# CenekAlbl/mvus

Hardware: AMD Instinct MI355X
Metric: residuals/sec (higher is better)
Workload: dtype f64; 1 GPU; BASELINE configs[2]: 32 cams x 504399 obs (504399 per GPU), rolling shutter on, 5003 spline control points, 15297 params, 1008798 residual rows; step = 1 trust-region trial (residual+Jacobian, LM normal equations + Schur solve, trial residual); solver=lm, parallelism=time-shard x1

## Files before the change

### mvus_amd/csrc/ba_rcs.hip.h

```cpp
#pragma once

namespace mvus {

constexpr int kRcsSP = 9;
constexpr int kRcsFactorThreads = 64 * (kRcsSP + 3);
constexpr int kRcsTrsmWaves = 4;

struct RcsView {
  double* Simg;
  double* Tsc;
  double* x;
  int nn, nbk;
};

__host__ __device__ __forceinline__ long long rcs_blk(int i, int j) { return ((long long)i * (i + 1) / 2 + j) * 256; }
__host__ __device__ inline size_t rcs_doubles(int nn) { const int nbk = (nn + 15) / 16; return (size_t)rcs_blk(nbk + 1, 0); }
__device__ __forceinline__ bcr_d4 rcs_load(const double* __restrict__ p) { return *reinterpret_cast<const bcr_d4*>(p); }
__device__ __forceinline__ void rcs_store(double* __restrict__ p, bcr_d4 v) { *reinterpret_cast<bcr_d4*>(p) = v; }
__device__ __forceinline__ bcr_d4 rcs_mma(bcr_d4 p, bcr_d4 q, bcr_d4 acc) {
#pragma unroll
  for (int s = 0; s < 4; ++s) acc = __builtin_amdgcn_mfma_f64_16x16x4f64(p[s], q[s], acc, 0, 0, 0);
  return acc;
}
__device__ __forceinline__ bcr_d4 rcs_matvec(bcr_d4 img, double w) {
  bcr_d4 out;
#pragma unroll
  for (int r = 0; r < 4; ++r) {
    double v = img[r] * w;
    v += dpp_shift<0x111, 0xF>(v, 0.0);
    v += dpp_shift<0x112, 0xF>(v, 0.0);
    v += dpp_shift<0x114, 0xF>(v, 0.0);
    v += dpp_shift<0x118, 0xF>(v, 0.0);
    out[r] = v;
  }
  return out;
}

struct RcsPivotChain { double d, r, e; bool bad; };
template <int J> __device__ __forceinline__ double rcs_bcast(double v) {
  const int lo = __builtin_amdgcn_mov_dpp(__double2loint(v), 0x150 + J, 0xf, 0xf, true);
  const int hi = __builtin_amdgcn_mov_dpp(__double2hiint(v), 0x150 + J, 0xf, 0xf, true);
  return __hiloint2double(hi, lo);
}
template <int STAGE, int J> __device__ __forceinline__ void rcs_chain_stage(RcsPivotChain& c, const double (&a)[16]) {
  if constexpr (STAGE == 0) { double d = rcs_bcast<J>(a[J]); c.bad |= !(d > 0.0); c.d = d > 0.0 ? d : 1.0; }
  else if constexpr (STAGE == 1) c.r = __builtin_amdgcn_rcp(c.d);
  else if constexpr (STAGE == 2 || STAGE == 4) c.e = 2.0 - c.d * c.r;
  else if constexpr (STAGE == 3 || STAGE == 5) c.r = c.r * c.e;
}
template <int FROM, int KN> struct RcsChainRest {
  static __device__ __forceinline__ void run(RcsPivotChain& c, const double (&a)[16]) {
    if constexpr (FROM <= 5) { rcs_chain_stage<FROM, KN>(c, a); RcsChainRest<FROM + 1, KN>::run(c, a); }
  }
};
template <int K, int J> struct RcsColOps {
  static __device__ __forceinline__ void run(double (&a)[16], double (&x)[16], double ta, double tx, double m, RcsPivotChain& c) {
    if constexpr (J < 16) {
      double mn = 0.0;
      if constexpr (J + 1 < 16) mn = rcs_bcast<J + 1>(a[K]);
      a[J] -= ta * m;
      x[J] -= tx * m;
      rcs_chain_stage<J - (K + 1), K + 1>(c, a);
      asm volatile("" : "+v"(a[J]), "+v"(x[J]), "+v"(c.d), "+v"(c.r), "+v"(c.e), "+v"(mn));
      __builtin_amdgcn_sched_barrier(0);
      RcsColOps<K, J + 1>::run(a, x, ta, tx, mn, c);
    }
  }
};
template <int K> struct RcsCols {
  static __device__ __forceinline__ void run(double (&a)[16], double (&x)[16], double (&rd)[16], RcsPivotChain& c) {
    const double r = c.r;
    rd[K] = r;
    if constexpr (K + 1 < 16) {
      const double m0 = rcs_bcast<K + 1>(a[K]);
      const double ta = a[K] * r, tx = x[K] * r;
      RcsColOps<K, K + 1>::run(a, x, ta, tx, m0, c);
      RcsChainRest<(15 - K < 6 ? 15 - K : 6), K + 1>::run(c, a);
      __builtin_amdgcn_sched_barrier(0);
      RcsCols<K + 1>::run(a, x, rd, c);
    }
  }
};
__device__ __forceinline__ void rcs_ldl16(double (&a)[16], double (&x)[16], double (&rd)[16], int lane, int* __restrict__ fail) {
  RcsPivotChain c{0.0, 0.0, 0.0, false};
  RcsChainRest<0, 0>::run(c, a);
  RcsCols<0>::run(a, x, rd, c);
  if (c.bad && lane == 0) fail[0] = 2;
}

__global__ __launch_bounds__(256) void k_rcs_finish(NEView ne, int ncols, int nslab, double lambda, const double* __restrict__ Gp, RcsView rv,
                                                    unsigned* __restrict__ flags) {
  constexpr int kT = 32, kRowsPer = 4, kRowStep = 8;
  const int r0 = threadIdx.x / kT, c = threadIdx.x % kT;
  const int b = blockIdx.x * kT + c;
  const long long stride = (long long)ne.CB * ncols;
  const int nn = ne.CB, npad = rv.nbk * 16;
  if (blockIdx.y == gridDim.y - 1) {
    if (blockIdx.x == 0 && threadIdx.x == 0) flags[0] = 0u;
    if (r0 != 0 || b >= npad) return;
    double gr = 0.0;
    if (b < nn) {
      for (int sl = 0; sl < nslab; sl += 8) {
        double t[8];
#pragma unroll
        for (int u = 0; u < 8; ++u) t[u] = sl + u < nslab ? Gp[(sl + u) * stride + (long long)b * ncols + ne.CB] : 0.0;
#pragma unroll
        for (int u = 0; u < 8; ++u) gr += t[u];
      }
    }
    const double val = b < nn ? ne.gc[b] - gr : 0.0;
    double* blk = rv.Simg + rcs_blk(rv.nbk, b / 16);
    const int cc = b % 16;
    for (int lr = 0; lr < 16; ++lr) blk[((cc % 4) * 16 + lr) * 4 + cc / 4] = lr == 0 ? val : 0.0;
    return;
  }
  if (blockIdx.x > blockIdx.y) return;
  double gsum[kRowsPer];
  long long goff[kRowsPer];
#pragma unroll
  for (int q = 0; q < kRowsPer; ++q) {
    const int a = blockIdx.y * kT + r0 + kRowStep * q;
    const int hi = a / kGemmT >= b / kGemmT ? a : b, lo = a / kGemmT >= b / kGemmT ? b : a;
    goff[q] = (a < nn && b < nn) ? (long long)hi * ncols + lo : -1;
    gsum[q] = 0.0;
  }
  for (int sl = 0; sl < nslab; sl += 8) {
    double t[8][kRowsPer];
#pragma unroll
    for (int u = 0; u < 8; ++u)
#pragma unroll
      for (int q = 0; q < kRowsPer; ++q) t[u][q] = (sl + u < nslab && goff[q] >= 0) ? Gp[(sl + u) * stride + goff[q]] : 0.0;
#pragma unroll
    for (int u = 0; u < 8; ++u)
#pragma unroll
      for (int q = 0; q < kRowsPer; ++q) gsum[q] += t[u][q];
  }
#pragma unroll
  for (int q = 0; q < kRowsPer; ++q) {
    const int a = blockIdx.y * kT + r0 + kRowStep * q;
    if (a >= npad || b >= npad || a / 16 < b / 16) continue;
    double v = a == b ? 1.0 : 0.0;
    if (a < nn && b < nn) {
      v = -gsum[q];
      if (a / ne.B == b / ne.B) {
        const int cam = a / ne.B;
        double h = ne.A[((long long)cam * ne.B + a % ne.B) * ne.B + b % ne.B];
        if (a == b) h += lambda * (h > 0.0 ? h : 1.0);
        v += h;
      }
    }
    const int cc = b % 16;
    rv.Simg[rcs_blk(a / 16, b / 16) + ((cc % 4) * 16 + a % 16) * 4 + cc / 4] = v;
  }
}

using rcs_u4 = __attribute__((ext_vector_type(4))) unsigned;
struct RcsWide { rcs_u4 a, b; };
__device__ __forceinline__ __amdgpu_buffer_rsrc_t rcs_rsrc(double* p, size_t doubles) {
  return __builtin_amdgcn_make_buffer_rsrc(p, 0, (int)(doubles * sizeof(double)), 0x00020000);
}
__device__ __forceinline__ void rcs_store_sc1(__amdgpu_buffer_rsrc_t r, long long dbl_off, bcr_d4 v) {
  RcsWide w;
  __builtin_memcpy(&w, &v, sizeof(w));
  __builtin_amdgcn_raw_buffer_store_b128(w.a, r, (int)(dbl_off * 8), 0, 16);
  __builtin_amdgcn_raw_buffer_store_b128(w.b, r, (int)(dbl_off * 8 + 16), 0, 16);
}
__device__ __forceinline__ bcr_d4 rcs_load_sc1(__amdgpu_buffer_rsrc_t r, long long dbl_off) {
  RcsWide w;
  w.a = __builtin_amdgcn_raw_buffer_load_b128(r, (int)(dbl_off * 8), 0, 16);
  w.b = __builtin_amdgcn_raw_buffer_load_b128(r, (int)(dbl_off * 8 + 16), 0, 16);
  bcr_d4 v;
  __builtin_memcpy(&v, &w, sizeof(v));
  return v;
}
__device__ __forceinline__ double rcs_load1_sc1(__amdgpu_buffer_rsrc_t r, long long dbl_off) {
  using u2 = __attribute__((ext_vector_type(2))) unsigned;
  const u2 w = __builtin_amdgcn_raw_buffer_load_b64(r, (int)(dbl_off * 8), 0, 16);
  double v;
  __builtin_memcpy(&v, &w, sizeof(v));
  return v;
}
__device__ __forceinline__ void rcs_store1_sc1(__amdgpu_buffer_rsrc_t r, long long dbl_off, double v) {
  using u2 = __attribute__((ext_vector_type(2))) unsigned;
  u2 w;
  __builtin_memcpy(&w, &v, sizeof(w));
  __builtin_amdgcn_raw_buffer_store_b64(w, r, (int)(dbl_off * 8), 0, 16);
}
constexpr unsigned kRcsSpinLimit = 1u << 21;
constexpr int kFailHandover = kFailHandoverCode;

template <int J> struct RcsXtTimes {
  static __device__ __forceinline__ double run(const double* __restrict__ col, double w, double acc) {
    if constexpr (J < 16) return RcsXtTimes<J + 1>::run(col, w, acc + col[J] * rcs_bcast<J>(w));
    else return acc;
  }
};
__device__ __forceinline__ double rcs_xt_times(const double* __restrict__ col, double w) { return RcsXtTimes<0>::run(col, w, 0.0); }
__device__ __forceinline__ void rcs_part_product(const bcr_d4 (&sl)[kRcsSP], int k, const double* __restrict__ xi, double* __restrict__ out, int lr, int lk) {
  const double xv = xi[lr];
#pragma unroll
  for (int kk = 0; kk < kRcsSP; ++kk) {
    if (kk != k) continue;
    const bcr_d4 y = rcs_matvec(sl[kk], xv);
    if (lr == 15) {
#pragma unroll
      for (int r = 0; r < 4; ++r) out[lk + 4 * r] = y[r];
    }
  }
}

__device__ __forceinline__ void rcs_pivot_role(int nc, int* __restrict__ fail, double* __restrict__ Dm, double* __restrict__ Xb, double* __restrict__ rdb) {
  const int lane = threadIdx.x & 63;
  __builtin_amdgcn_s_setprio(3);
  for (int k = 0; k < nc; ++k) {
    if (k == 0) lds_barrier();
    double a[16], x[16], rd[16];
    int lr = lane & 15;
    asm volatile("" : "+v"(lr));
#pragma unroll
    for (int j = 0; j < 16; ++j) {
      a[j] = Dm[lr * 17 + j];
      x[j] = j == lr ? 1.0 : 0.0;
    }
    rcs_ldl16(a, x, rd, lane, fail);
    if (lane < 16) {
#pragma unroll
      for (int q = 0; q < 4; ++q) rcs_store(Xb + k * 256 + lane * 16 + 4 * q, bcr_d4{x[4 * q], x[4 * q + 1], x[4 * q + 2], x[4 * q + 3]});
    }
    if (lane == 0) {
#pragma unroll
      for (int q = 0; q < 4; ++q) rcs_store(rdb + k * 16 + 4 * q, bcr_d4{rd[4 * q], rd[4 * q + 1], rd[4 * q + 2], rd[4 * q + 3]});
    }
    lds_barrier();
    lds_barrier();
  }
}

__device__ __forceinline__ void rcs_trsm_role(RcsView rv, int c0, int nc, unsigned* __restrict__ flags, int* __restrict__ fail, double* __restrict__ xch,
                                              int* __restrict__ abort_s, unsigned spin_limit) {
  const int lane = threadIdx.x & 63, wave = __builtin_amdgcn_readfirstlane(threadIdx.x >> 6), lk = lane >> 4;
  const int c1 = c0 + nc, gi = c1 + (int)blockIdx.x - 1;
  const size_t tot = rcs_doubles(rv.nn);
  const __amdgpu_buffer_rsrc_t rS = rcs_rsrc(rv.Simg, tot), rT = rcs_rsrc(rv.Tsc, tot);
  constexpr int kSlots = (kRcsSP + kRcsTrsmWaves - 1) / kRcsTrsmWaves;
  bcr_d4 s[kSlots];
  const bcr_d4 zero{0.0, 0.0, 0.0, 0.0};
#pragma unroll
  for (int u = 0; u < kSlots; ++u) {
    const int jl = wave + kRcsTrsmWaves * u;
    s[u] = jl < nc ? rcs_load(rv.Simg + rcs_blk(gi, c0 + jl) + lane * 4) : zero;
  }
  if (threadIdx.x == 0) *abort_s = 0;
  lds_barrier();
#pragma unroll
  for (int k = 0; k < kRcsSP; ++k) {
    if (k >= nc) continue;
    if (threadIdx.x == 0 && *abort_s == 0) {
      const unsigned want = (unsigned)(c0 * 16 + k + 1);
      unsigned spins = 0;
      while (__hip_atomic_load(flags, __ATOMIC_RELAXED, __HIP_MEMORY_SCOPE_AGENT) < want) {
        __builtin_amdgcn_s_sleep(8);
        if (++spins > spin_limit) { *abort_s = 1; fail[0] = kFailHandover; fail[2] = 1; break; }
      }
    }
    lds_barrier();
    const bool dead = *abort_s != 0;
    bcr_d4 tj[kSlots];
    bool up[kSlots];
#pragma unroll
    for (int u = 0; u < kSlots; ++u) {
      const int jl = wave + kRcsTrsmWaves * u;
      up[u] = jl > k && jl < nc && !dead;
      tj[u] = up[u] ? rcs_load_sc1(rS, rcs_blk(c0 + jl, c0 + k) + lane * 4) : zero;
    }
    if (wave == k % kRcsTrsmWaves && !dead) {
      const bcr_d4 xi = rcs_load_sc1(rS, rcs_blk(c0 + k, c0 + k) + lane * 4);
      bcr_d4 nrd;
#pragma unroll
      for (int r = 0; r < 4; ++r) nrd[r] = -rcs_load1_sc1(rT, rcs_blk(c0 + k, c0 + k) + lk + 4 * r);
      const bcr_d4 t = rcs_mma(xi, s[k / kRcsTrsmWaves], zero);
      s[k / kRcsTrsmWaves] = t;
      rcs_store(xch + (k & 1) * 256 + lane * 4, t * nrd);
    }
    lds_barrier();
    if (k + 1 >= nc || dead) continue;
    const bcr_d4 sc = rcs_load(xch + (k & 1) * 256 + lane * 4);
#pragma unroll
    for (int q = 0; q < 4; ++q)
#pragma unroll
      for (int u = 0; u < kSlots; ++u)
        if (up[u]) s[u] = __builtin_amdgcn_mfma_f64_16x16x4f64(tj[u][q], sc[q], s[u], 0, 0, 0);
  }
#pragma unroll
  for (int u = 0; u < kSlots; ++u) {
    const int jl = wave + kRcsTrsmWaves * u;
    if (jl >= nc) continue;
    bcr_d4 sc;
#pragma unroll
    for (int r = 0; r < 4; ++r) sc[r] = -rcs_load1_sc1(rT, rcs_blk(c0 + jl, c0 + jl) + lk + 4 * r) * s[u][r];
    rcs_store(rv.Simg + rcs_blk(gi, c0 + jl) + lane * 4, s[u]);
    rcs_store(rv.Tsc + rcs_blk(gi, c0 + jl) + lane * 4, sc);
  }
}

__device__ __forceinline__ void rcs_publisher_role(RcsView rv, int c0, int nc, unsigned* __restrict__ flags, const double* __restrict__ Xb,
                                                   const double* __restrict__ rdb, const double* __restrict__ panel) {
  const int lane = threadIdx.x & 63, lr = lane & 15, lk = lane >> 4;
  const size_t tot = rcs_doubles(rv.nn);
  const __amdgpu_buffer_rsrc_t rS = rcs_rsrc(rv.Simg, tot), rT = rcs_rsrc(rv.Tsc, tot);
  lds_barrier();
  for (int k = 0; k < nc; ++k) {
    lds_barrier();
    if (k > 0) {
      asm volatile("s_waitcnt vmcnt(0)" ::: "memory");
      if (lane == 0) __hip_atomic_store(flags, (unsigned)(c0 * 16 + k), __ATOMIC_RELAXED, __HIP_MEMORY_SCOPE_AGENT);
    }
    lds_barrier();
    bcr_d4 xi;
#pragma unroll
    for (int r = 0; r < 4; ++r) xi[r] = Xb[k * 256 + (lk + 4 * r) * 16 + lr];
    rcs_store_sc1(rS, rcs_blk(c0 + k, c0 + k) + lane * 4, xi);
    if (lane < 16) rcs_store1_sc1(rT, rcs_blk(c0 + k, c0 + k) + lane, rdb[k * 16 + lane]);
    for (int jl = k + 1; jl < nc; ++jl) rcs_store_sc1(rS, rcs_blk(c0 + jl, c0 + k) + lane * 4, rcs_load(panel + jl * 256 + lane * 4));
    asm volatile("s_waitcnt lgkmcnt(0)" ::: "memory");
  }
  asm volatile("s_waitcnt vmcnt(0)" ::: "memory");
  if (lane == 0) __hip_atomic_store(flags, (unsigned)(c0 * 16 + nc), __ATOMIC_RELAXED, __HIP_MEMORY_SCOPE_AGENT);
}

__global__ __launch_bounds__(kRcsFactorThreads) void k_rcs_factor(RcsView rv, int c0, int* __restrict__ fail, int last, double* __restrict__ pc,
                                                                  unsigned* __restrict__ flags, unsigned spin_limit) {
  __shared__ double Dm[16 * 17];
  __shared__ __attribute__((aligned(32))) double Xb[kRcsSP * 256];
  __shared__ __attribute__((aligned(32))) double rdb[kRcsSP * 16];
  __shared__ __attribute__((aligned(32))) double panel[(kRcsSP + 1) * 256];
  __shared__ int abort_s;
  const int lane = threadIdx.x & 63, wave = __builtin_amdgcn_readfirstlane(threadIdx.x >> 6), lr = lane & 15, lk = lane >> 4;
  const int nc = min(kRcsSP, rv.nbk - c0), R = rv.nbk;
  if (blockIdx.x > 0) {
    if (wave < kRcsTrsmWaves) rcs_trsm_role(rv, c0, nc, flags, fail, panel, &abort_s, spin_limit);
    return;
  }
  if (wave == kRcsSP + 2) {
    if (gridDim.x > 1) rcs_publisher_role(rv, c0, nc, flags, Xb, rdb, panel);
    else { lds_barrier(); for (int k = 0; k < nc; ++k) { lds_barrier(); lds_barrier(); } }
    if (last) { lds_barrier(); for (int i = 0; i < nc; ++i) { lds_barrier(); lds_barrier(); } }
    return;
  }
  __shared__ double u0[kRcsSP * 16];
  __shared__ double part[kRcsSP * kRcsSP * 16];
  __shared__ double xs[kRcsSP * 16];
  if (wave == kRcsSP + 1) {
    rcs_pivot_role(nc, fail, Dm, Xb, rdb);
    if (!last || c0 > 0)
      for (int k = 0; k < nc; ++k) {
        bcr_d4 xi;
#pragma unroll
        for (int r = 0; r < 4; ++r) xi[r] = Xb[k * 256 + (lk + 4 * r) * 16 + lr];
        rcs_store(rv.Simg + rcs_blk(c0 + k, c0 + k) + lane * 4, xi);
        if (lane < 16) rv.Tsc[rcs_blk(c0 + k, c0 + k) + lane] = rdb[k * 16 + lane];
      }
    if (!last) return;
    __builtin_amdgcn_s_setprio(0);
    lds_barrier();
    for (int i = nc - 1; i >= 0; --i) {
      double xi = 0.0;
      if (lane < 16) {
        double w = u0[i * 16 + lane];
        for (int ip = i + 1; ip < nc; ++ip) w -= part[(ip * kRcsSP + i) * 16 + lane];
        w *= rdb[i * 16 + lane];
        xi = rcs_xt_times(Xb + i * 256 + lane * 16, w);
        xs[i * 16 + lane] = xi;
      }
      lds_barrier();
      lds_barrier();
    }
    if (lane < 16)
      for (int k = 0; k < nc; ++k) {
        const int a = (c0 + k) * 16 + lane;
        const double v = xs[k * 16 + lane];
        rv.x[a] = v;
        if (a < rv.nn) pc[a] = -v;
      }
    return;
  }
  const int il = wave;
  const bool has = il <= nc, isR = il == nc;
  const int gi = isR ? R : c0 + il;
  bcr_d4 sl[kRcsSP];
  const bcr_d4 zero{0.0, 0.0, 0.0, 0.0};
#pragma unroll
  for (int jl = 0; jl < kRcsSP; ++jl) sl[jl] = (has && jl < nc && (isR || jl <= il)) ? rcs_load(rv.Simg + rcs_blk(gi, c0 + jl) + lane * 4) : zero;
  if (wave == 0) {
#pragma unroll
    for (int r = 0; r < 4; ++r) Dm[(lk + 4 * r) * 17 + lr] = sl[0][r];
  }
  lds_barrier();
#pragma unroll
  for (int k = 0; k < kRcsSP; ++k) {
    if (k < nc) {
      lds_barrier();
      const bool act = has && il > k;
      const bool owner = act && il == k + 1 && !isR && k + 1 < nc;
      if (owner) __builtin_amdgcn_s_setprio(2);
      bcr_d4 sc = zero;
      if (act) {
        bcr_d4 xi;
#pragma unroll
        for (int r = 0; r < 4; ++r) xi[r] = Xb[k * 256 + (lk + 4 * r) * 16 + lr];
        const bcr_d4 t = rcs_mma(xi, sl[k], zero);
        sl[k] = t;
#pragma unroll
        for (int r = 0; r < 4; ++r) sc[r] = -rdb[k * 16 + lk + 4 * r] * t[r];
        rcs_store(panel + il * 256 + lane * 4, t);
      }
      const int kn = k + 1 < kRcsSP ? k + 1 : 0;
      if (owner) {
        sl[kn] = rcs_mma(sl[k], sc, sl[kn]);
#pragma unroll
        for (int r = 0; r < 4; ++r) Dm[(lk + 4 * r) * 17 + lr] = sl[kn][r];
        __builtin_amdgcn_s_setprio(0);
      }
      lds_barrier();
      {
        bcr_d4 tj[kRcsSP];
        bool up[kRcsSP];
#pragma unroll
        for (int jl = k + 1; jl < kRcsSP; ++jl) {
          up[jl] = jl < nc && act && (isR || jl <= il) && !(owner && jl == k + 1);
          tj[jl] = up[jl] ? rcs_load(panel + jl * 256 + lane * 4) : zero;
        }
#pragma unroll
        for (int q = 0; q < 4; ++q)
#pragma unroll
          for (int jl = k + 1; jl < kRcsSP; ++jl)
            if (up[jl]) sl[jl] = __builtin_amdgcn_mfma_f64_16x16x4f64(tj[jl][q], sc[q], sl[jl], 0, 0, 0);
      }
    }
  }
  if (has && (!last || c0 > 0)) {
#pragma unroll
  for (int k = 0; k < kRcsSP; ++k) {
    if (k < nc && il > k) {
      bcr_d4 sc;
#pragma unroll
      for (int r = 0; r < 4; ++r) sc[r] = -rdb[k * 16 + lk + 4 * r] * sl[k][r];
      rcs_store(rv.Simg + rcs_blk(gi, c0 + k) + lane * 4, sl[k]);
      rcs_store(rv.Tsc + rcs_blk(gi, c0 + k) + lane * 4, sc);
    }
  }
  }
  if (!last) return;
  if (has && isR && lr == 0) {
#pragma unroll
    for (int k = 0; k < kRcsSP; ++k)
      if (k < nc)
#pragma unroll
        for (int r = 0; r < 4; ++r) u0[k * 16 + lk + 4 * r] = sl[k][r];
  }
  lds_barrier();
  for (int i = nc - 1; i >= 0; --i) {
    const bool mine = has && !isR && il > i;
    int kd = mine ? 2 * i - il : -1;
    if (kd >= 0) rcs_part_product(sl, kd, xs + il * 16, part + (il * kRcsSP + kd) * 16, lr, lk);
    lds_barrier();
    kd = (has && !isR && il == i) ? i - 1 : (mine ? 2 * i - il - 1 : -1);
    if (kd >= 0) rcs_part_product(sl, kd, xs + il * 16, part + (il * kRcsSP + kd) * 16, lr, lk);
    lds_barrier();
  }
}

__host__ __device__ inline int rcs_stage_doubles(int nc) { return nc * 256 + nc * 16 + nc * (nc - 1) / 2 * 256; }
__device__ __forceinline__ int rcs_tri(int j, int k) { return j * (j - 1) / 2 + k; }
template <int NWAVES>
__device__ __forceinline__ void rcs_stage(const RcsView& rv, int c0, int nc, double* __restrict__ st, int lane, int wave) {
  constexpr int kMaxBlk = kRcsSP + kRcsSP * (kRcsSP - 1) / 2, kPer = (kMaxBlk + NWAVES - 1) / NWAVES;
  double* rds = st + nc * 256;
  double* ts = rds + nc * 16;
  const int nblk = nc + nc * (nc - 1) / 2;
  bcr_d4 v[kPer];
  double rdv[kPer];
  int dst[kPer];
#pragma unroll
  for (int u = 0; u < kPer; ++u) {
    const int t = wave + NWAVES * u;
    dst[u] = -1; rdv[u] = 0.0;
    if (t < nc) {
      v[u] = rcs_load(rv.Simg + rcs_blk(c0 + t, c0 + t) + lane * 4);
      if (lane < 16) rdv[u] = rv.Tsc[rcs_blk(c0 + t, c0 + t) + lane];
      dst[u] = t * 256;
    } else if (t < nblk) {
      const int e = t - nc;
      int j = (int)((1.0f + sqrtf(1.0f + 8.0f * (float)e)) * 0.5f);
      while (j * (j - 1) / 2 > e) --j;
      while (j * (j + 1) / 2 <= e) ++j;
      const int k = e - j * (j - 1) / 2;
      v[u] = rcs_load(rv.Simg + rcs_blk(c0 + j, c0 + k) + lane * 4);
      dst[u] = (int)(ts - st) + e * 256;
    }
  }
#pragma unroll
  for (int u = 0; u < kPer; ++u) {
    const int t = wave + NWAVES * u;
    if (dst[u] >= 0) rcs_store(st + dst[u] + lane * 4, v[u]);
    if (t < nc && lane < 16) rds[t * 16 + lane] = rdv[u];
  }
}

__global__ __launch_bounds__(64 * kRcsTrsmWaves) void k_rcs_trsm(RcsView rv, int c0) {
  extern __shared__ __attribute__((aligned(32))) double rcs_lds[];
  const int lane = threadIdx.x & 63, wave = __builtin_amdgcn_readfirstlane(threadIdx.x >> 6), lk = lane >> 4;
  const int nc = min(kRcsSP, rv.nbk - c0), c1 = c0 + nc;
  rcs_stage<kRcsTrsmWaves>(rv, c0, nc, rcs_lds, lane, wave);
  const double* rds = rcs_lds + nc * 256;
  const double* ts = rds + nc * 16;
  double* xch = rcs_lds + rcs_stage_doubles(nc);
  const int gi = c1 + blockIdx.x;
  constexpr int kSlots = (kRcsSP + kRcsTrsmWaves - 1) / kRcsTrsmWaves;
  bcr_d4 s[kSlots];
  const bcr_d4 zero{0.0, 0.0, 0.0, 0.0};
#pragma unroll
  for (int u = 0; u < kSlots; ++u) {
    const int jl = wave + kRcsTrsmWaves * u;
    s[u] = jl < nc ? rcs_load(rv.Simg + rcs_blk(gi, c0 + jl) + lane * 4) : zero;
  }
  lds_barrier();
#pragma unroll
  for (int k = 0; k < kRcsSP; ++k) {
    if (k >= nc) continue;
    if (wave == k % kRcsTrsmWaves) {
      const bcr_d4 t = rcs_mma(rcs_load(rcs_lds + k * 256 + lane * 4), s[k / kRcsTrsmWaves], zero);
      s[k / kRcsTrsmWaves] = t;
      bcr_d4 sc;
#pragma unroll
      for (int r = 0; r < 4; ++r) sc[r] = -rds[k * 16 + lk + 4 * r] * t[r];
      rcs_store(xch + (k & 1) * 256 + lane * 4, sc);
    }
    lds_barrier();
    if (k + 1 >= nc) continue;
    const bcr_d4 sc = rcs_load(xch + (k & 1) * 256 + lane * 4);
    bcr_d4 tj[kSlots];
    bool up[kSlots];
#pragma unroll
    for (int u = 0; u < kSlots; ++u) {
      const int jl = wave + kRcsTrsmWaves * u;
      up[u] = jl > k && jl < nc;
      tj[u] = up[u] ? rcs_load(ts + rcs_tri(jl, k) * 256 + lane * 4) : zero;
    }
#pragma unroll
    for (int q = 0; q < 4; ++q)
#pragma unroll
      for (int u = 0; u < kSlots; ++u)
        if (up[u]) s[u] = __builtin_amdgcn_mfma_f64_16x16x4f64(tj[u][q], sc[q], s[u], 0, 0, 0);
  }
#pragma unroll
  for (int u = 0; u < kSlots; ++u) {
    const int jl = wave + kRcsTrsmWaves * u;
    if (jl >= nc) continue;
    bcr_d4 sc;
#pragma unroll
    for (int r = 0; r < 4; ++r) sc[r] = -rds[jl * 16 + lk + 4 * r] * s[u][r];
    rcs_store(rv.Simg + rcs_blk(gi, c0 + jl) + lane * 4, s[u]);
    rcs_store(rv.Tsc + rcs_blk(gi, c0 + jl) + lane * 4, sc);
  }
}

__global__ __launch_bounds__(256) void k_rcs_syrk(RcsView rv, int c0) {
  const int lane = threadIdx.x & 63, wave = __builtin_amdgcn_readfirstlane(threadIdx.x >> 6);
  const int nc = min(kRcsSP, rv.nbk - c0), c1 = c0 + nc, m = rv.nbk - c1;
  const int t = blockIdx.x * 4 + wave, ntri = m * (m + 1) / 2;
  if (t >= ntri + m) return;
  int il, jl;
  if (t < ntri) {
    il = (int)((sqrt(8.0 * t + 1.0) - 1.0) * 0.5);
    while ((il + 1) * (il + 2) / 2 <= t) ++il;
    while (il * (il + 1) / 2 > t) --il;
    jl = t - il * (il + 1) / 2;
  } else { il = m; jl = t - ntri; }
  const int gi = c1 + il, gj = c1 + jl;
  double* blk = rv.Simg + rcs_blk(gi, gj) + lane * 4;
  bcr_d4 acc = rcs_load(blk);
  bcr_d4 pj[kRcsSP], qi[kRcsSP];
#pragma unroll
  for (int k = 0; k < kRcsSP; ++k) {
    if (k >= nc) continue;
    pj[k] = rcs_load(rv.Simg + rcs_blk(gj, c0 + k) + lane * 4);
    qi[k] = rcs_load(rv.Tsc + rcs_blk(gi, c0 + k) + lane * 4);
  }
#pragma unroll
  for (int k = 0; k < kRcsSP; ++k)
    if (k < nc) acc = rcs_mma(pj[k], qi[k], acc);
  rcs_store(blk, acc);
}

constexpr int kRcsBackWaves = 16;
__host__ __device__ inline int rcs_backsub_doubles(int nbk) { return nbk * 16 + (1 + kRcsBackWaves) * kRcsSP * 16 + rcs_stage_doubles(kRcsSP); }
__global__ __launch_bounds__(64 * kRcsBackWaves) void k_rcs_backsub(RcsView rv, double* __restrict__ pc, int Kfirst) {
  extern __shared__ __attribute__((aligned(32))) double rcs_lds[];
  const int lane = threadIdx.x & 63, wave = __builtin_amdgcn_readfirstlane(threadIdx.x >> 6), lr = lane & 15, lk = lane >> 4;
  const int nbk = rv.nbk, R = nbk;
  double* xs = rcs_lds;
  double* u = xs + nbk * 16;
  double* up = u + kRcsSP * 16;
  double* st = up + kRcsBackWaves * kRcsSP * 16;
  for (int a = (Kfirst + 1) * kRcsSP * 16 + threadIdx.x; a < nbk * 16; a += 64 * kRcsBackWaves) xs[a] = rv.x[a];
  constexpr int kBatch = 4;
  for (int K = Kfirst; K >= 0; --K) {
    const int c0 = K * kRcsSP, nc = min(kRcsSP, nbk - c0), c1 = c0 + nc;
    lds_barrier();
    double* rds = st + nc * 256;
    double* ts = rds + nc * 16;
    const int nblk = nc + nc * (nc - 1) / 2;
    constexpr int kPer = (kRcsSP + kRcsSP * (kRcsSP - 1) / 2 + kRcsBackWaves - 1) / kRcsBackWaves;
    bcr_d4 sv[kPer];
    double srd[kPer];
    int sdst[kPer];
#pragma unroll
    for (int q = 0; q < kPer; ++q) {
      const int t = wave + kRcsBackWaves * q;
      sdst[q] = -1; srd[q] = 0.0;
      if (t < nc) {
        sv[q] = rcs_load(rv.Simg + rcs_blk(c0 + t, c0 + t) + lane * 4);
        if (lane < 16) srd[q] = rv.Tsc[rcs_blk(c0 + t, c0 + t) + lane];
        sdst[q] = t * 256;
      } else if (t < nblk) {
        const int e = t - nc;
        int j = (int)((1.0f + sqrtf(1.0f + 8.0f * (float)e)) * 0.5f);
        while (j * (j - 1) / 2 > e) --j;
        while (j * (j + 1) / 2 <= e) ++j;
        sv[q] = rcs_load(rv.Simg + rcs_blk(c0 + j, c0 + e - j * (j - 1) / 2) + lane * 4);
        sdst[q] = (int)(ts - st) + e * 256;
      }
    }
    double tR = 0.0;
    if (threadIdx.x < nc * 16) {
      const int jl = threadIdx.x / 16, row = threadIdx.x % 16;
      tR = rv.Simg[rcs_blk(R, c0 + jl) + ((row & 3) * 16) * 4 + (row >> 2)];
    }
    const int nitem = (nbk - c1) * nc;
    bcr_d4 img[kBatch];
    double xv[kBatch];
#pragma unroll
    for (int q = 0; q < kBatch; ++q) {
      const int it = min(wave + kRcsBackWaves * q, max(nitem - 1, 0)), i = c1 + it / nc, jl = it % nc;
      img[q] = nitem > 0 ? rcs_load(rv.Simg + rcs_blk(i, c0 + jl) + lane * 4) : bcr_d4{0.0, 0.0, 0.0, 0.0};
      xv[q] = nitem > 0 ? xs[i * 16 + lr] : 0.0;
    }
#pragma unroll
    for (int q = 0; q < kPer; ++q) {
      const int t = wave + kRcsBackWaves * q;
      if (sdst[q] >= 0) rcs_store(st + sdst[q] + lane * 4, sv[q]);
      if (t < nc && lane < 16) rds[t * 16 + lane] = srd[q];
    }
    for (int e = lane; e < nc * 16; e += 64) up[wave * kRcsSP * 16 + e] = 0.0;
    lds_wave_sync();
    for (int it0 = wave; it0 < nitem; it0 += kRcsBackWaves * kBatch) {
      if (it0 != wave) {
#pragma unroll
        for (int q = 0; q < kBatch; ++q) {
          const int it = min(it0 + kRcsBackWaves * q, nitem - 1), i = c1 + it / nc, jl = it % nc;
          img[q] = rcs_load(rv.Simg + rcs_blk(i, c0 + jl) + lane * 4);
          xv[q] = xs[i * 16 + lr];
        }
      }
#pragma unroll
      for (int q = 0; q < kBatch; ++q) {
        const int it = it0 + kRcsBackWaves * q;
        if (it >= nitem) continue;
        const int jl = it % nc;
        const bcr_d4 y = rcs_matvec(img[q], xv[q]);
        if (lr == 15) {
#pragma unroll
          for (int r = 0; r < 4; ++r) up[wave * kRcsSP * 16 + jl * 16 + lk + 4 * r] += y[r];
        }
      }
    }
    lds_barrier();
    if (threadIdx.x < nc * 16) {
      double v = tR;
#pragma unroll
      for (int w = 0; w < kRcsBackWaves; ++w) v -= up[w * kRcsSP * 16 + threadIdx.x];
      u[threadIdx.x] = v;
    }
    lds_barrier();
    for (int k = nc - 1; k >= 0; --k) {
      if (wave == 0) {
        const bcr_d4 y = rcs_matvec(rcs_load(st + k * 256 + lane * 4), rds[k * 16 + lr] * u[k * 16 + lr]);
        if (lr == 15) {
#pragma unroll
          for (int r = 0; r < 4; ++r) xs[(c0 + k) * 16 + lk + 4 * r] = y[r];
        }
      }
      lds_barrier();
      if (wave < k) {
        const bcr_d4 y = rcs_matvec(rcs_load(ts + rcs_tri(k, wave) * 256 + lane * 4), xs[(c0 + k) * 16 + lr]);
        if (lr == 15) {
#pragma unroll
          for (int r = 0; r < 4; ++r) u[wave * 16 + lk + 4 * r] -= y[r];
        }
      }
      lds_barrier();
    }
  }
  const int top = min((Kfirst + 1) * kRcsSP * 16, rv.nn);
  for (int a = threadIdx.x; a < top; a += 64 * kRcsBackWaves) pc[a] = -xs[a];
}

}
```

Measured before the change: 1.132 billion residuals/s.

## Move next-pivot diagonal update into pivot wave and remap wave roles across SIMDs

```diff
diff --git a/mvus_amd/csrc/ba_rcs.hip.h b/mvus_amd/csrc/ba_rcs.hip.h
--- a/mvus_amd/csrc/ba_rcs.hip.h
+++ b/mvus_amd/csrc/ba_rcs.hip.h
@@ -209,8 +209,10 @@
   }
 }
 
-__device__ __forceinline__ void rcs_pivot_role(int nc, int* __restrict__ fail, double* __restrict__ Dm, double* __restrict__ Xb, double* __restrict__ rdb) {
-  const int lane = threadIdx.x & 63;
+__device__ __forceinline__ void rcs_pivot_role(int nc, int* __restrict__ fail, double* __restrict__ Dm, double* __restrict__ Xb, double* __restrict__ rdb,
+                                               const double* __restrict__ stg, double* __restrict__ panel) {
+  const int lane = threadIdx.x & 63, lk = lane >> 4;
+  const bcr_d4 zero{0.0, 0.0, 0.0, 0.0};
   __builtin_amdgcn_s_setprio(3);
   for (int k = 0; k < nc; ++k) {
     if (k == 0) lds_barrier();
@@ -232,6 +234,20 @@
       for (int q = 0; q < 4; ++q) rcs_store(rdb + k * 16 + 4 * q, bcr_d4{rd[4 * q], rd[4 * q + 1], rd[4 * q + 2], rd[4 * q + 3]});
     }
     lds_barrier();
+    if (k + 1 < nc) {
+      const int lc = lane & 15;
+      bcr_d4 xi, sc;
+#pragma unroll
+      for (int r = 0; r < 4; ++r) xi[r] = Xb[k * 256 + (lk + 4 * r) * 16 + lc];
+      const bcr_d4 u = rcs_load(stg + lane * 4), dn = rcs_load(stg + 256 + lane * 4);
+      const bcr_d4 t = rcs_mma(xi, u, zero);
+#pragma unroll
+      for (int r = 0; r < 4; ++r) sc[r] = -rdb[k * 16 + lk + 4 * r] * t[r];
+      rcs_store(panel + (k + 1) * 256 + lane * 4, t);
+      const bcr_d4 d = rcs_mma(t, sc, dn);
+#pragma unroll
+      for (int r = 0; r < 4; ++r) Dm[(lk + 4 * r) * 17 + lc] = d[r];
+    }
     lds_barrier();
   }
 }
@@ -328,19 +344,44 @@
   if (lane == 0) __hip_atomic_store(flags, (unsigned)(c0 * 16 + nc), __ATOMIC_RELAXED, __HIP_MEMORY_SCOPE_AGENT);
 }
 
+__device__ __forceinline__ int rcs_factor_role(int* __restrict__ simd_of) {
+  constexpr int kWaves = kRcsSP + 3;
+  constexpr int kRole[kWaves] = {kRcsSP + 1, kRcsSP + 2, 0, kRcsSP, 5, 1, 8, 4, 3, 7, 6, 2};
+  static_assert(kRcsSP == 9, "the role table is written for super-panels of nine block columns");
+  const int wave = __builtin_amdgcn_readfirstlane(threadIdx.x >> 6);
+  const int simd = __builtin_amdgcn_readfirstlane((__builtin_amdgcn_s_getreg((1 << 11) | (4 << 6) | 4)) & 3);
+  if ((threadIdx.x & 63) == 0) simd_of[wave] = simd;
+  lds_barrier();
+  bool three = true;
+  int rank = 0;
+#pragma unroll
+  for (int s = 0; s < 4; ++s) {
+    int c = 0;
+#pragma unroll
+    for (int w = 0; w < kWaves; ++w) c += simd_of[w] == s;
+    three &= c == 3;
+  }
+#pragma unroll
+  for (int w = 0; w < kWaves; ++w) rank += (w < wave && simd_of[w] == simd);
+  return __builtin_amdgcn_readfirstlane(three ? kRole[simd * 3 + rank] : wave);
+}
+
 __global__ __launch_bounds__(kRcsFactorThreads) void k_rcs_factor(RcsView rv, int c0, int* __restrict__ fail, int last, double* __restrict__ pc,
                                                                   unsigned* __restrict__ flags, unsigned spin_limit) {
   __shared__ double Dm[16 * 17];
   __shared__ __attribute__((aligned(32))) double Xb[kRcsSP * 256];
   __shared__ __attribute__((aligned(32))) double rdb[kRcsSP * 16];
   __shared__ __attribute__((aligned(32))) double panel[(kRcsSP + 1) * 256];
+  __shared__ __attribute__((aligned(32))) double stg[2 * 256];
   __shared__ int abort_s;
-  const int lane = threadIdx.x & 63, wave = __builtin_amdgcn_readfirstlane(threadIdx.x >> 6), lr = lane & 15, lk = lane >> 4;
+  __shared__ int simd_of[kRcsSP + 3];
+  const int lane = threadIdx.x & 63, lr = lane & 15, lk = lane >> 4;
   const int nc = min(kRcsSP, rv.nbk - c0), R = rv.nbk;
   if (blockIdx.x > 0) {
-    if (wave < kRcsTrsmWaves) rcs_trsm_role(rv, c0, nc, flags, fail, panel, &abort_s, spin_limit);
+    if (__builtin_amdgcn_readfirstlane(threadIdx.x >> 6) < kRcsTrsmWaves) rcs_trsm_role(rv, c0, nc, flags, fail, panel, &abort_s, spin_limit);
     return;
   }
+  const int wave = rcs_factor_role(simd_of);
   if (wave == kRcsSP + 2) {
     if (gridDim.x > 1) rcs_publisher_role(rv, c0, nc, flags, Xb, rdb, panel);
     else { lds_barrier(); for (int k = 0; k < nc; ++k) { lds_barrier(); lds_barrier(); } }
@@ -351,7 +392,7 @@
   __shared__ double part[kRcsSP * kRcsSP * 16];
   __shared__ double xs[kRcsSP * 16];
   if (wave == kRcsSP + 1) {
-    rcs_pivot_role(nc, fail, Dm, Xb, rdb);
+    rcs_pivot_role(nc, fail, Dm, Xb, rdb, stg, panel);
     if (!last || c0 > 0)
       for (int k = 0; k < nc; ++k) {
         bcr_d4 xi;
@@ -399,10 +440,14 @@
 #pragma unroll
   for (int k = 0; k < kRcsSP; ++k) {
     if (k < nc) {
+      const int kn = k + 1 < kRcsSP ? k + 1 : 0;
+      const bool owner = has && il == k + 1 && !isR && k + 1 < nc;
+      if (owner) {
+        rcs_store(stg + lane * 4, sl[k]);
+        rcs_store(stg + 256 + lane * 4, sl[kn]);
+      }
       lds_barrier();
-      const bool act = has && il > k;
-      const bool owner = act && il == k + 1 && !isR && k + 1 < nc;
-      if (owner) __builtin_amdgcn_s_setprio(2);
+      const bool act = has && il > k && !owner;
       bcr_d4 sc = zero;
       if (act) {
         bcr_d4 xi;
@@ -414,20 +459,14 @@
         for (int r = 0; r < 4; ++r) sc[r] = -rdb[k * 16 + lk + 4 * r] * t[r];
         rcs_store(panel + il * 256 + lane * 4, t);
       }
-      const int kn = k + 1 < kRcsSP ? k + 1 : 0;
-      if (owner) {
-        sl[kn] = rcs_mma(sl[k], sc, sl[kn]);
-#pragma unroll
-        for (int r = 0; r < 4; ++r) Dm[(lk + 4 * r) * 17 + lr] = sl[kn][r];
-        __builtin_amdgcn_s_setprio(0);
-      }
       lds_barrier();
+      if (owner) sl[k] = rcs_load(panel + il * 256 + lane * 4);
       {
         bcr_d4 tj[kRcsSP];
         bool up[kRcsSP];
 #pragma unroll
         for (int jl = k + 1; jl < kRcsSP; ++jl) {
-          up[jl] = jl < nc && act && (isR || jl <= il) && !(owner && jl == k + 1);
+          up[jl] = jl < nc && act && (isR || jl <= il);
           tj[jl] = up[jl] ? rcs_load(panel + jl * 256 + lane * 4) : zero;
         }
 #pragma unroll
```

Result: no change. 1.142 billion residuals/s, median of 6 (+0.9%).
